# matchylabs/matchy

Hardware: AMD Instinct MI355X
Metric: log GB/s scanned (matchy match hot path, 100K IoCs) (higher is better)
Workload: dtype u8

## Files before the change

### matchy_amd/csrc/validate_kernels.hip

```cpp
#include <hip/hip_runtime.h>

#include <cstdlib>

#include "hashes.h"
#include "scan_types.h"

#include "device_shared.h"

namespace mxy {


struct BackReader {
    const uint8_t* p;
    uint32_t pos;
    uint32_t cb;
    uint32_t k;
    uint64_t cur, nxt;
    __device__ __forceinline__ static uint64_t load8(const uint8_t* a) { uint64_t v; __builtin_memcpy(&v, a, 8); return v; }
    __device__ __forceinline__ void init(const uint8_t* base, uint32_t q) {
        p = base; pos = q; cb = 0; k = 0; cur = 0; nxt = 0;
        if (q >= 16) { cb = q - 8; k = 8; cur = load8(p + cb); nxt = load8(p + cb - 8); }
    }
    __device__ __forceinline__ uint32_t next() {
        --pos;
        if (pos < 16) return p[pos];
        if (k == 0) { cur = nxt; cb -= 8; k = 8; nxt = cb >= 8 ? load8(p + cb - 8) : 0ull; }
        const uint32_t c = (uint32_t)(cur >> 56);
        cur <<= 8;
        --k;
        return c;
    }
};

struct WalkInit {
    uint64_t rh;
    uint32_t cur = 0, last_c = 0, labels = 1;
    bool high = false, bad = false, found = false;
};
struct WalkState { uint32_t pos, cur, last_c, labels; bool high, bad, found; };
constexpr int WALK_NO = 0, WALK_YES = 1, WALK_LONG = 2;
constexpr uint32_t WALK_BUDGET_WORDS = 128;
template <bool HASH>
__device__ __forceinline__ int domain_walk_back(const LogView& lg, const DevDb& db, uint32_t min_labels, uint32_t e, BackReader& br,
                                                 const WalkInit& wi, uint32_t& start, WalkState* long_out, bool* defer_utf8 = nullptr,
                                                 bool* hit_start = nullptr) {
    uint64_t rh = wi.rh;
    bool found = wi.found, bad = wi.bad, high = wi.high;
    uint32_t labels = wi.labels, cur = wi.cur, last_c = wi.last_c;
    uint32_t first_c = 0x100;
    uint32_t words = 0;
    while (br.pos > 0) {
        if ((!HASH || found) && br.pos >= 32 && (cur != 0 || last_c == '.')) {
            constexpr uint64_t H = 0x8080808080808080ull;
            uint32_t pos = br.pos;
            uint64_t w = BackReader::load8(lg.p + pos - 8);
            bool any = false;
            for (;;) {
                const uint64_t wn = pos >= 24 ? BackReader::load8(lg.p + pos - 16) : 0ull;
                const ByteMasks m = domain_masks(w);
                if ((~m.dc & H) != 0) break;
                const uint64_t dr = (m.dot >> 8) | (last_c == '.' ? (0x80ull << 56) : 0ull);
                const uint64_t sr = (m.dash >> 8) | (last_c == '-' ? (0x80ull << 56) : 0ull);
                if (((m.dot & (dr | sr)) | (m.dash & dr)) != 0) bad = true;
                if (m.dot != 0 && !bad) found = true;
                labels += (uint32_t)__popcll(m.dot);
                high |= m.high != 0;
                last_c = (uint32_t)w & 0xFF;
                cur = last_c == '.' ? 0u : 1u;
                pos -= 8;
                any = true;
                if (pos < 24) break;
                if (long_out && ++words >= WALK_BUDGET_WORDS) {
                    *long_out = WalkState{pos, cur, last_c, labels, high, bad, found};
                    return WALK_LONG;
                }
                w = wn;
            }
            if (any) { br.init(lg.p, pos); continue; }
        }
        uint32_t c = br.next();
        if (!d_is_domain_char_fast(c)) { first_c = c; ++br.pos; break; }
        if (HASH && !found && e - br.pos - 1 > db.max_suffix_len) return WALK_NO;
        if (c == '.') {
            if (cur == 0 || last_c == '-') bad = true;
            if (HASH) { if (!found && !bad) found = psl_contains(db, psl_hash_finish(rh), lg.p + br.pos + 1, e - br.pos - 1); }
            else if (!bad) found = true;
            ++labels;
            cur = 0;
        } else {
            if (cur == 0 && c == '-') bad = true;
            ++cur;
            high |= c >= 0x80;
        }
        if (HASH) rh = psl_hash_step(rh, (uint8_t)c);
        last_c = c;
    }
    const uint32_t s = br.pos;
    if (hit_start && first_c == 0x100) *hit_start = true;
    if (cur == 0 || last_c == '-') bad = true;
    if (bad || !found || labels < min_labels) return WALK_NO;
    if (first_c != 0x100 && !d_is_boundary(first_c)) return WALK_NO;
    if (high && defer_utf8) *defer_utf8 = true;
    else if (high && !d_valid_utf8(lg.p + s, e - s)) return WALK_NO;
    start = s;
    return WALK_YES;
}

__device__ __forceinline__ bool coop_valid_utf8(const uint8_t* p, uint32_t n) {
    const uint32_t lane = lane_id();
    uint64_t carry = 0;
    uint32_t c2 = 0;
    bool ok = true;
    for (uint32_t base = 0; base < n; base += 64) {
        const uint32_t b = base + lane < n ? p[base + lane] : 0u;
        const uint64_t cont = __ballot((b & 0xC0u) == 0x80u);
        const uint64_t l2 = __ballot(b >= 0xC2u && b <= 0xDFu), l3 = __ballot((b & 0xF0u) == 0xE0u), l4 = __ballot(b >= 0xF0u && b <= 0xF4u);
        const uint64_t badb = __ballot(b == 0xC0u || b == 0xC1u || b >= 0xF5u);
        const uint64_t e0 = __ballot(b == 0xE0u), ed = __ballot(b == 0xEDu), f0 = __ballot(b == 0xF0u), f4 = __ballot(b == 0xF4u);
        const uint64_t ltA0 = __ballot(b < 0xA0u), gt9F = __ballot(b > 0x9Fu), lt90 = __ballot(b < 0x90u), gt8F = __ballot(b > 0x8Fu);
        const uint64_t lead = l2 | l3 | l4, lead34 = l3 | l4;
        const uint64_t exp = (lead << 1) | (lead34 << 2) | (l4 << 3) | carry;
        carry = (lead >> 63) | (lead34 >> 62) | (l4 >> 61);
        uint64_t bad2 = ((e0 << 1) & ltA0) | ((ed << 1) & gt9F) | ((f0 << 1) & lt90) | ((f4 << 1) & gt8F);
        if (c2 & 1) bad2 |= ltA0 & 1; if (c2 & 2) bad2 |= gt9F & 1; if (c2 & 4) bad2 |= lt90 & 1; if (c2 & 8) bad2 |= gt8F & 1;
        c2 = (uint32_t)(e0 >> 63) | ((uint32_t)(ed >> 63) << 1) | ((uint32_t)(f0 >> 63) << 2) | ((uint32_t)(f4 >> 63) << 3);
        if ((exp ^ cont) | badb | bad2) { ok = false; break; }
    }
    return ok && carry == 0;
}

__device__ __forceinline__ void coop_domain_skip(const LogView& lg, WalkState& st) {
    constexpr uint64_t H = 0x8080808080808080ull;
    const uint32_t lane = lane_id();
    while (st.pos >= 512 + 32) {
        const uint32_t base = st.pos - 512;
        const uint64_t w = BackReader::load8(lg.p + base + 8 * lane);
        const ByteMasks m = domain_masks(w);
        const uint64_t stop = __ballot((~m.dc & H) != 0);
        const int hi = stop ? 63 - (int)__clzll((long long)stop) : -1;
        const bool valid = (int)lane > hi;
        uint32_t nb = (uint32_t)__shfl_down((int)((uint32_t)w & 0xFFu), 1);
        if (lane == 63) nb = st.last_c;
        const uint64_t dr = (m.dot >> 8) | (nb == '.' ? (0x80ull << 56) : 0ull);
        const uint64_t sr = (m.dash >> 8) | (nb == '-' ? (0x80ull << 56) : 0ull);
        const bool badl = ((m.dot & (dr | sr)) | (m.dash & dr)) != 0;
        if (__ballot(valid && badl)) st.bad = true;
        if (__ballot(valid && m.dot != 0) && !st.bad) st.found = true;
        if (__ballot(valid && m.high != 0)) st.high = true;
        uint32_t nd = valid ? (uint32_t)__popcll(m.dot) : 0u;
#pragma unroll
        for (int off = 32; off > 0; off >>= 1) nd += (uint32_t)__shfl_xor((int)nd, off);
        st.labels += nd;
        const uint32_t low = (uint32_t)w & 0xFFu;
        if (hi >= 0) {
            if (hi < 63) {
                st.pos = base + 8 * (uint32_t)(hi + 1);
                st.last_c = (uint32_t)__shfl((int)low, hi + 1);
                st.cur = st.last_c == '.' ? 0u : 1u;
            }
            return;
        }
        st.pos = base;
        st.last_c = (uint32_t)__shfl((int)low, 0);
        st.cur = st.last_c == '.' ? 0u : 1u;
    }
}

struct DomLong { WalkState st; uint32_t e; bool alone; };
__device__ int val_domain(const LogView& lg, const DevDb& db, const uint32_t* bloom, const uint2* tldtab, uint32_t min_labels,
                          uint32_t j, uint32_t& start, uint32_t& end, DomLong* long_out, bool* edge = nullptr) {
    uint32_t p = j, th = 2166136261u;
    bool open = true;
    uint32_t stop_c = 0x100;
    uint2 w = make_uint2(0u, 0u);
    const bool wide = j + 8 <= lg.len;
    if (wide) {
        __builtin_memcpy(&w, lg.p + j, 8);
#pragma unroll
        for (int k = 0; k < 8; ++k) {
            if (open) {
                const uint32_t c = ((k < 4 ? w.x : w.y) >> (8 * (k & 3))) & 0xFF;
                if (!d_is_domain_char_fast(c)) { open = false; stop_c = c; }
                else {
                    if (c == '.') return false;
                    th = tld_hash_step(th, c);
                    ++p;
                }
            }
        }
    }
    while (open && p < lg.len) {
        uint32_t c = lg.at(p);
        if (!d_is_domain_char_fast(c)) { stop_c = c; break; }
        if (c == '.') return false;
        if (p - j >= db.max_tld_len) return false;
        th = tld_hash_step(th, c);
        ++p;
    }
    const uint32_t e = p, ll = e - j;
    if (edge && stop_c == 0x100) *edge = true;
    if (ll > db.max_tld_len) return false;
    if (stop_c != 0x100 && !d_is_boundary(stop_c)) return false;
    bool alone = false;
    if (wide && ll <= 7) {
        const uint32_t lo = ll >= 4 ? w.x : (w.x & ((1u << (8 * ll)) - 1u));
        const uint32_t hi = ll > 4 ? (w.y & ((1u << (8 * (ll - 4))) - 1u)) : 0u;
        uint32_t slot = tld_tab_slot(lo, hi);
        for (;;) {
            const uint2 t = tldtab[slot];
            if ((t.y >> 24) == 0) return false;
            if (t.x == lo && (t.y & 0xFFFFFFu) == hi) { alone = (t.y >> 24) & 1; break; }
            slot = (slot + 1) & ((1u << TLD_TAB_BITS) - 1);
        }
    } else {
        const uint32_t bit = tld_hash_bit(th);
        if (!((bloom[bit >> 5] >> (bit & 31)) & 1)) return false;
    }
    uint32_t s;
    BackReader br;
    br.init(lg.p, e);
    WalkInit wi;
    wi.rh = psl_hash_init();
    WalkState ws{};
    const int r = alone ? domain_walk_back<false>(lg, db, min_labels, e, br, wi, s, long_out ? &ws : nullptr, nullptr, edge)
                        : domain_walk_back<true>(lg, db, min_labels, e, br, wi, s, long_out ? &ws : nullptr, nullptr, edge);
    if (r == WALK_LONG) { long_out->st = ws; long_out->e = e; long_out->alone = alone; return WALK_LONG; }
    if (r != WALK_YES) return WALK_NO;
    start = s; end = e;
    return WALK_YES;
}
__device__ bool val_domain_resume(const LogView& lg, const DevDb& db, uint32_t min_labels, const DomLong& dl, uint32_t& start, uint32_t& end, bool& need_utf8) {
    BackReader br;
    br.init(lg.p, dl.st.pos);
    WalkInit wi;
    wi.rh = psl_hash_init();
    wi.cur = dl.st.cur; wi.last_c = dl.st.last_c; wi.labels = dl.st.labels; wi.high = dl.st.high; wi.bad = dl.st.bad; wi.found = dl.st.found;
    uint32_t s;
    if (domain_walk_back<false>(lg, db, min_labels, dl.e, br, wi, s, nullptr, &need_utf8) != WALK_YES) return false;
    start = s; end = dl.e;
    return true;
}

__device__ __forceinline__ int val_domain_pre(const uint2* tldtab, uint32_t min_labels, uint32_t j, uint2 w, uint64_t b0, uint64_t b1,
                                              uint64_t b2, uint32_t& start, uint32_t& end) {
    constexpr uint64_t H = 0x8080808080808080ull;
    const uint64_t w64 = (uint64_t)w.x | ((uint64_t)w.y << 32);
    const ByteMasks mw = domain_masks(w64);
    const uint64_t ndc = ~mw.dc & H;
    const uint32_t ll = ndc ? (uint32_t)(__ffsll((long long)ndc) - 1) >> 3 : 8u;
    if (ll <= 7 && ll >= 1) {
        const uint64_t below = (1ull << (8 * ll)) - 1ull;
        if (mw.dot & below) return 0;
        const uint32_t stop_c = (uint32_t)(w64 >> (8 * ll)) & 0xFF;
        if (!d_is_boundary(stop_c)) return 0;
        const uint32_t lo = (uint32_t)(w64 & below), hi = (uint32_t)((w64 & below) >> 32);
        uint32_t slot = tld_tab_slot(lo, hi);
        bool alone = false;
        for (;;) {
            const uint2 t = tldtab[slot];
            if ((t.y >> 24) == 0) return 0;
            if (t.x == lo && (t.y & 0xFFFFFFu) == hi) { alone = (t.y >> 24) & 1; break; }
            slot = (slot + 1) & ((1u << TLD_TAB_BITS) - 1);
        }
        if (alone) {
            const ByteMasks m0 = domain_masks(b0), m1 = domain_masks(b1), m2 = domain_masks(b2);
            const uint64_t n0m = ~m0.dc & H, n1m = ~m1.dc & H, n2m = ~m2.dc & H;
            const uint32_t c0 = n0m ? (uint32_t)__clzll((long long)n0m) >> 3 : 8u;
            const uint32_t c1 = n1m ? (uint32_t)__clzll((long long)n1m) >> 3 : 8u, c2 = n2m ? (uint32_t)__clzll((long long)n2m) >> 3 : 8u;
            const uint32_t consumed = c0 < 8 ? c0 : (c1 < 8 ? 8 + c1 : 16 + c2);
            if (consumed < 24 || j == 24) {
                auto top = [](uint32_t k) -> uint64_t { return k == 0 ? 0ull : (~0ull << (64 - 8 * k)); };
                const uint64_t r0 = top(min(consumed, 8u)), r1 = top(consumed > 8 ? min(consumed - 8, 8u) : 0u),
                               r2 = top(consumed > 16 ? consumed - 16 : 0u);
                const uint64_t d0 = m0.dot >> 8, d1 = (m1.dot >> 8) | (m0.dot << 56), d2 = (m2.dot >> 8) | (m1.dot << 56);
                const uint64_t s0 = m0.dash >> 8, s1 = (m1.dash >> 8) | (m0.dash << 56), s2 = (m2.dash >> 8) | (m1.dash << 56);
                const uint64_t bad = ((m0.dot & (d0 | s0)) | (m0.dash & d0)) & r0;
                const uint64_t bad1 = ((m1.dot & (d1 | s1)) | (m1.dash & d1)) & r1, bad2 = ((m2.dot & (d2 | s2)) | (m2.dash & d2)) & r2;
                const uint32_t ndots = (uint32_t)(__popcll(m0.dot & r0) + __popcll(m1.dot & r1) + __popcll(m2.dot & r2));
                const uint32_t li = 24 - consumed;
                const uint64_t lw = li < 8 ? b2 : li < 16 ? b1 : b0;
                const uint32_t left_c = (uint32_t)(lw >> (8 * (li & 7))) & 0xFF;
                const uint32_t fi = 23 - consumed;
                const uint64_t fw = fi < 8 ? b2 : fi < 16 ? b1 : b0;
                const uint32_t first_c = consumed < 24 ? (uint32_t)(fw >> (8 * (fi & 7))) & 0xFF : 0x100u;
                const uint32_t lastc = (uint32_t)(w64 >> (8 * (ll - 1))) & 0xFF;
                const bool any_bad = (bad | bad1 | bad2) != 0 || lastc == '-' || consumed == 0 || left_c == '.' || left_c == '-';
                if (any_bad || ndots == 0 || 1 + ndots < min_labels) return 0;
                if (first_c != 0x100 && !d_is_boundary(first_c)) return 0;
                const uint32_t s_pos = j - consumed;
                const bool high = ((m0.high & r0) | (m1.high & r1) | (m2.high & r2) | (mw.high & below)) != 0;
                if (high) return 2;
                start = s_pos; end = j + ll;
                return 1;
            }
        }
    }
    return 2;
}

template <int NB>
__device__ __forceinline__ int val_domain_ctx(const uint2* tldtab, uint32_t min_labels, uint32_t j, uint2 w, const uint64_t (&b)[NB],
                                              uint32_t& start, uint32_t& end) {
    static_assert(NB >= 1 && NB <= 7, "a label must not reach 64 bytes inside the context");
    constexpr uint64_t H = 0x8080808080808080ull;
    const uint64_t w64 = (uint64_t)w.x | ((uint64_t)w.y << 32);
    const ByteMasks mw = domain_masks(w64);
    const uint64_t ndc = ~mw.dc & H;
    const uint32_t ll = ndc ? (uint32_t)(__ffsll((long long)ndc) - 1) >> 3 : 8u;
    if (ll > 7 || ll < 1) return 2;
    const uint64_t below = (1ull << (8 * ll)) - 1ull;
    if (mw.dot & below) return 0;
    const uint32_t stop_c = (uint32_t)(w64 >> (8 * ll)) & 0xFF;
    if (!d_is_boundary(stop_c)) return 0;
    const uint32_t lo = (uint32_t)(w64 & below), hi = (uint32_t)((w64 & below) >> 32);
    uint32_t slot = tld_tab_slot(lo, hi);
    bool alone = false;
    for (;;) {
        const uint2 t = tldtab[slot];
        if ((t.y >> 24) == 0) return 0;
        if (t.x == lo && (t.y & 0xFFFFFFu) == hi) { alone = (t.y >> 24) & 1; break; }
        slot = (slot + 1) & ((1u << TLD_TAB_BITS) - 1);
    }
    if (!alone) return 2;
    ByteMasks m[NB];
    uint32_t consumed = 0;
    bool open = true;
#pragma unroll
    for (int k = 0; k < NB; ++k) {
        m[k] = domain_masks(b[k]);
        const uint64_t nm = ~m[k].dc & H;
        const uint32_t ck = nm ? (uint32_t)__clzll((long long)nm) >> 3 : 8u;
        if (open) { consumed += ck; open = ck == 8; }
    }
    if (consumed == 8 * NB && j != 8 * NB) return 2;
    uint64_t bad = 0, high = mw.high & below;
    uint32_t ndots = 0;
#pragma unroll
    for (int k = 0; k < NB; ++k) {
        const uint32_t in_k = consumed > 8u * k ? min(consumed - 8u * k, 8u) : 0u;
        const uint64_t r = in_k == 0 ? 0ull : (~0ull << (64 - 8 * in_k));
        const uint64_t d = (m[k].dot >> 8) | (k ? (m[k ? k - 1 : 0].dot << 56) : 0ull);
        const uint64_t sd = (m[k].dash >> 8) | (k ? (m[k ? k - 1 : 0].dash << 56) : 0ull);
        bad |= ((m[k].dot & (d | sd)) | (m[k].dash & d)) & r;
        ndots += (uint32_t)__popcll(m[k].dot & r);
        high |= m[k].high & r;
    }
    const uint32_t li = 8 * NB - consumed, fi = li - 1;
    uint32_t left_c = 0, first_c = 0x100u;
#pragma unroll
    for (int k = 0; k < NB; ++k) {
        const uint32_t wi = (uint32_t)(NB - 1 - k);
        if ((li >> 3) == wi) left_c = (uint32_t)(b[k] >> (8 * (li & 7))) & 0xFF;
        if (consumed < 8 * NB && (fi >> 3) == wi) first_c = (uint32_t)(b[k] >> (8 * (fi & 7))) & 0xFF;
    }
    const uint32_t lastc = (uint32_t)(w64 >> (8 * (ll - 1))) & 0xFF;
    const bool any_bad = bad != 0 || lastc == '-' || consumed == 0 || left_c == '.' || left_c == '-';
    if (any_bad || ndots == 0 || 1 + ndots < min_labels) return 0;
    if (first_c != 0x100u && !d_is_boundary(first_c)) return 0;
    if (high) return 2;
    start = j - consumed; end = j + ll;
    return 1;
}

__device__ bool all_hex(const LogView& lg, uint32_t s, uint32_t n) {
    for (uint32_t k = 0; k < n; ++k) if (!d_is_hex(lg.at(s + k))) return false;
    return true;
}
__device__ __forceinline__ bool hex4(uint32_t x) {
    const uint32_t t = x & 0x7F7F7F7Fu, l = t | 0x20202020u;
    const uint32_t dig = (t + 0x50505050u) & ~(t + 0x46464646u);
    const uint32_t alp = (l + 0x1F1F1F1Fu) & ~(l + 0x19191919u);
    return (((dig | alp) & ~x) & 0x80808080u) == 0x80808080u;
}
__device__ __forceinline__ bool all_hex_wide(const uint8_t* p, uint32_t n) {
    bool ok = true;
#pragma unroll 4
    for (uint32_t k = 0; k < n; k += 8) {
        uint2 v;
        __builtin_memcpy(&v, p + k, 8);
        ok = ok && hex4(v.x) && hex4(v.y);
    }
    return ok;
}


__device__ __forceinline__ uint32_t d_lower(uint32_t c) { return (c - 'A' < 26u) ? c + 32 : c; }

__device__ bool val_ipv6(const LogView& lg, uint32_t p2, uint32_t& start, uint32_t& end) {
    uint32_t s = p2 - 1;
    while (s > 0) { uint32_t c = lg.at(s - 1); if (!d_is_hex(c) && c != ':') break; --s; }
    uint32_t e = p2 + 1;
    while (e < lg.len) { uint32_t c = lg.at(e); if (!d_is_hex(c) && c != ':') break; ++e; }
    uint32_t n = e - s;
    if (n < 8 || n > 64) return false;
    const uint8_t* c = lg.p + s;
    if ((c[0] == ':' && c[1] == ':') || (c[n - 2] == ':' && c[n - 1] == ':')) return false;
    if (d_lower(c[0]) == 'f' && d_lower(c[1]) == 'e') { uint32_t x = d_lower(c[2]); if (x == '8' || x == '9' || x == 'a' || x == 'b') return false; }
    uint16_t seg[8];
    if (!d_parse_ipv6(c, n, seg)) return false;
    start = s; end = e;
    return true;
}

__device__ bool val_ipv6_win(const uint8_t* win, uint32_t p2, uint32_t& start, uint32_t& end) {
    uint32_t s = 39;
    while (s > 0) { uint32_t c = win[s - 1]; if (!d_is_hex(c) && c != ':') break; --s; }
    if (s == 0) return false;
    uint32_t e = 41;
    while (e < 80) { uint32_t c = win[e]; if (!d_is_hex(c) && c != ':') break; ++e; }
    if (e == 80) return false;
    const uint32_t n = e - s;
    if (n < 8 || n > 64) return false;
    const uint8_t* c = win + s;
    if ((c[0] == ':' && c[1] == ':') || (c[n - 2] == ':' && c[n - 1] == ':')) return false;
    if (d_lower(c[0]) == 'f' && d_lower(c[1]) == 'e') { uint32_t x = d_lower(c[2]); if (x == '8' || x == '9' || x == 'a' || x == 'b') return false; }
    uint16_t seg[8];
    if (!d_parse_ipv6(c, n, seg)) return false;
    start = p2 - 40 + s; end = p2 - 40 + e;
    return true;
}

struct LocalMasks { uint64_t loc, dot, alp; };
struct LocalMasks32 { uint32_t loc, dot, alp; };
__device__ __forceinline__ LocalMasks32 email_local_masks32(uint32_t x) {
    constexpr uint32_t H = 0x80808080u, L7 = 0x7F7F7F7Fu;
    const uint32_t t = x & L7, l = t | 0x20202020u;
    const uint32_t dig = (t + 0x50505050u) & ~(t + 0x46464646u);
    const uint32_t alp = (l + 0x1F1F1F1Fu) & ~(l + 0x05050505u);
    const uint32_t ndot = (t ^ 0x2E2E2E2Eu) + L7, ndash = (t ^ 0x2D2D2D2Du) + L7;
    const uint32_t nus = (t ^ 0x5F5F5F5Fu) + L7, npl = (t ^ 0x2B2B2B2Bu) + L7;
    LocalMasks32 m;
    m.dot = ~ndot & ~x & H;
    m.alp = alp & ~x & H;
    m.loc = (dig | alp | ~ndot | ~ndash | ~nus | ~npl) & ~x & H;
    return m;
}
__device__ __forceinline__ LocalMasks email_local_masks(uint64_t x) {
    const LocalMasks32 lo = email_local_masks32((uint32_t)x), hi = email_local_masks32((uint32_t)(x >> 32));
    LocalMasks m;
    m.loc = (uint64_t)lo.loc | ((uint64_t)hi.loc << 32);
    m.dot = (uint64_t)lo.dot | ((uint64_t)hi.dot << 32);
    m.alp = (uint64_t)lo.alp | ((uint64_t)hi.alp << 32);
    return m;
}
struct EmailState { uint32_t s, prev; bool has_letter, dotdot; };
__device__ __forceinline__ bool email_local_scan(const LogView& lg, EmailState& es, bool budget) {
    constexpr uint64_t H = 0x8080808080808080ull;
    uint32_t s = es.s, prev = es.prev, words = 0;
    bool has_letter = es.has_letter, dotdot = es.dotdot, is_long = false;
    if (s >= 32) {
        uint64_t w = BackReader::load8(lg.p + s - 8);
        for (;;) {
// ... 237 lines not shown
            const uint64_t t = bc[(i + 4) % 5] ^ rotl64(bc[(i + 1) % 5], 1);
#pragma unroll
            for (int j = 0; j < 25; j += 5) st[j + i] ^= t;
        }
        uint64_t t = st[1];
#pragma unroll
        for (int i = 0; i < 24; ++i) { const int j = PILN[i]; const uint64_t b = st[j]; st[j] = rotl64(t, ROTC[i]); t = b; }
#pragma unroll
        for (int j = 0; j < 25; j += 5) {
#pragma unroll
            for (int i = 0; i < 5; ++i) bc[i] = st[j + i];
#pragma unroll
            for (int i = 0; i < 5; ++i) st[j + i] ^= (~bc[(i + 1) % 5]) & bc[(i + 2) % 5];
        }
        st[0] ^= RC[round];
    }
    out[0] = st[0]; out[1] = st[1]; out[2] = st[2]; out[3] = st[3];
}

__device__ __forceinline__ int d_b58_val(uint32_t c) {
    if (c >= '1' && c <= '9') return (int)c - '1';
    if (c >= 'A' && c <= 'H') return (int)c - 'A' + 9;
    if (c >= 'J' && c <= 'N') return (int)c - 'J' + 17;
    if (c >= 'P' && c <= 'Z') return (int)c - 'P' + 22;
    if (c >= 'a' && c <= 'k') return (int)c - 'a' + 33;
    if (c >= 'm' && c <= 'z') return (int)c - 'm' + 44;
    return -1;
}
template <int NL>
__device__ uint32_t d_base58_decode(const uint8_t* s, uint32_t n, uint8_t* dec) {
    uint32_t L[NL];
#pragma unroll
    for (int i = 0; i < NL; ++i) L[i] = 0;
    uint32_t zeros = 0;
    bool leading = true;
    for (uint32_t k = 0; k < n; ++k) {
        const int v = d_b58_val(s[k]);
        if (v < 0) return 0;
        if (leading && v == 0) { ++zeros; continue; }
        leading = false;
        uint32_t carry = (uint32_t)v;
#pragma unroll
        for (int i = 0; i < NL; ++i) {
            const uint64_t t = (uint64_t)L[i] * 58u + carry;
            L[i] = (uint32_t)t;
            carry = (uint32_t)(t >> 32);
        }
    }
    uint32_t nbytes = 0;
#pragma unroll
    for (int i = 0; i < NL; ++i) if (L[i]) nbytes = 4 * i + 1 + ((31u - (uint32_t)__clz((int)L[i])) >> 3);
    for (uint32_t k = 0; k < zeros; ++k) dec[k] = 0;
#pragma unroll
    for (int i = 0; i < NL; ++i) {
#pragma unroll
        for (int bb = 0; bb < 4; ++bb) {
            const uint32_t j = 4 * i + bb;
            if (j < nbytes) dec[zeros + nbytes - 1 - j] = (uint8_t)(L[i] >> (8 * bb));
        }
    }
    return zeros + nbytes;
}
__device__ bool val_btc_base58(const uint8_t* s, uint32_t n, uint8_t* dec) {
    const uint32_t dl = d_base58_decode<12>(s, n, dec);
    if (dl < 5) return false;
    Sha256 h1, h2;
    h1.hash(dec, dl - 4);
    uint32_t w[16];
#pragma unroll
    for (int i = 0; i < 8; ++i) w[i] = h1.h[i];
    w[8] = 0x80000000u;
#pragma unroll
    for (int i = 9; i < 15; ++i) w[i] = 0;
    w[15] = 256;
    h2.init();
    h2.block(w);
    const uint32_t chk = ((uint32_t)dec[dl - 4] << 24) | ((uint32_t)dec[dl - 3] << 16) | ((uint32_t)dec[dl - 2] << 8) | dec[dl - 1];
    return h2.h[0] == chk;
}
__device__ bool val_monero(const uint8_t* s, uint32_t n, uint8_t* dec) {
    const uint32_t dl = d_base58_decode<21>(s, n, dec);
    if (dl < 5) return false;
    uint64_t h[4];
    d_keccak256_1blk(dec, dl - 4, h);
    const uint32_t chk = (uint32_t)dec[dl - 4] | ((uint32_t)dec[dl - 3] << 8) | ((uint32_t)dec[dl - 2] << 16) | ((uint32_t)dec[dl - 1] << 24);
    return (uint32_t)h[0] == chk;
}
__device__ int d_bech32_val(uint32_t c) {
    const char* CS = "qpzry9x8gf2tvdw0s3jn54khce6mua7l";
    for (int i = 0; i < 32; ++i) if ((uint32_t)CS[i] == c) return i;
    return -1;
}
__device__ bool val_btc_bech32(const uint8_t* s, uint32_t n) {
    if (n < 3 + 6) return false;
    auto step = [](uint32_t chk, uint32_t v) {
        const uint32_t GEN[5] = {0x3b6a57b2, 0x26508e6d, 0x1ea119fa, 0x3d4233dd, 0x2a1462b3};
        uint32_t top = chk >> 25;
        chk = ((chk & 0x1ffffff) << 5) ^ v;
        for (int i = 0; i < 5; ++i) if ((top >> i) & 1) chk ^= GEN[i];
        return chk;
    };
    uint32_t chk = 1;
    chk = step(chk, 'b' >> 5); chk = step(chk, 'c' >> 5); chk = step(chk, 0); chk = step(chk, 'b' & 31); chk = step(chk, 'c' & 31);
    for (uint32_t k = 3; k < n; ++k) {
        int v = d_bech32_val(s[k]);
        if (v < 0) return false;
        chk = step(chk, (uint32_t)v);
    }
    return chk == 1 || chk == 0x2bc830a3u;
}
__device__ bool val_eth(const uint8_t* a, uint8_t* lower) {
    bool all_lower = true, all_upper = true;
    for (int i = 0; i < 40; ++i) {
        uint32_t c = a[2 + i];
        if (!d_is_hex(c)) return false;
        if (d_is_alpha(c)) { if (c >= 'a') all_upper = false; else all_lower = false; }
        lower[i] = (uint8_t)d_lower(c);
    }
    if (all_lower || all_upper) return true;
    uint64_t h[4];
    d_keccak256_1blk(lower, 40, h);
    for (int i = 0; i < 40; ++i) {
        uint32_t c = a[2 + i];
        if (d_is_alpha(c)) {
            const uint32_t byte = (uint32_t)(h[i >> 4] >> (8 * ((i >> 1) & 7))) & 0xFF;
            const uint32_t nib = (i & 1) ? (byte & 0x0f) : (byte >> 4);
            if ((c < 'a') != (nib >= 8)) return false;
        }
    }
    return true;
}

template <int MODE>
__global__ __launch_bounds__(256) void k_validate_dom(TokParams p, DevDb db) {
    constexpr bool AC = MODE == 1, SFX = MODE == 2;
    __shared__ uint2 tldtab[1u << TLD_TAB_BITS];
    __shared__ __attribute__((aligned(16))) uint32_t strbuf[256][8];
    __shared__ uint8_t dcls[AC ? 256 : 4];
    __shared__ uint32_t drows[AC ? DFA_LDS_ENTRIES_VAL : 1];
    for (uint32_t i = threadIdx.x; i < (1u << TLD_TAB_BITS); i += blockDim.x) tldtab[i] = db.tld_tab[i];
    DfaView dv{dcls, drows, 0};
    if constexpr (AC) dv = dfa_stage<DFA_LDS_ENTRIES_VAL>(db, dcls, drows);
    __syncthreads();
    ChunkWriter<Candidate, CAND_CHUNK> cw_dense;
    __shared__ Candidate wb_cand[4][64];
    BufferedWriter<Candidate> cw(wb_cand[threadIdx.x >> 6]);
    __shared__ RareAnchor wb_slow[4][64];
    BufferedWriter<RareAnchor> sw(wb_slow[threadIdx.x >> 6]);
    const Candidate SC{0, 0xFFFFFFFFu, 0, 0};
    const uint32_t stride = gridDim.x * blockDim.x;
    const uint32_t nd = min(p.counters->n_dom, p.dom_cap);
    struct Rec { uint32_t j; uint32_t c[8]; };
    auto load_rec = [&](uint32_t i, Rec& r) {
        r.j = 0xFFFFFFFFu;
#pragma unroll
        for (int k = 0; k < 8; ++k) r.c[k] = 0;
        if (i < nd) {
            r.j = p.dom_list[dom_plane_index(i, 0)];
#pragma unroll
            for (int k = 0; k < 8; ++k) r.c[k] = p.dom_list[dom_plane_index(i, 1 + k)];
        }
    };
    Rec cur, nxt;
    load_rec(blockIdx.x * blockDim.x + threadIdx.x, cur);
    {
        uint32_t g = cur.j;
#pragma unroll
        for (int k = 0; k < 8; ++k) g ^= cur.c[k];
        asm volatile("" ::"v"(g));
    }
    uint32_t pend_start = 0, pend_lt = 0, pend_word = 0xFFFFFFFFu, pend_bit = 0, n_valid = 0;
    uint32_t pend_sw[SFX ? 4 : 1] = {0}, pend_sb[SFX ? 4 : 1] = {0};
    bool pend = false, pend_over = false;
    uint32_t* sb = strbuf[threadIdx.x];
    auto queue_glob = [&](uint32_t b, uint32_t n) {
        if (!p.glob_work_d) return;
        const uint32_t lane = lane_id();
        const bool g = lane < n && b + lane < p.cand_cap && cw.buf[lane].pad == CAND_GLOB;
        const uint64_t m = __ballot(g);
        if (!m) return;
        uint32_t wb = 0;
        if (lane == 0) wb = atomicAdd(&p.counters->n_glob_work_d, (uint32_t)__popcll(m));
        wb = __builtin_amdgcn_readfirstlane(wb);
        const uint32_t slot = wb + mbcnt64(m);
        if (g && slot < p.glob_work_d_cap) p.glob_work_d[slot] = b + lane;
    };
    auto emit_pending = [&]() {
        if (!p.filter_lit) { cw_dense.append(pend, Candidate{pend_start, pend_lt, 0u, 0u}, p.cands, p.cand_cap, p.n_cand, SC); return; }
        bool lit = (pend_word >> pend_bit) & 1;
        uint32_t flag = 0;
        if constexpr (SFX) {
            bool g = pend_over;
#pragma unroll
            for (int q = 0; q < 4; ++q) g = g || ((pend_sw[q] >> pend_sb[q]) & 1);
            flag = g ? CAND_GLOB : CAND_NO_GLOB;
            lit = lit || g;
        }
        if constexpr (AC) flag = pend_over ? CAND_GLOB : CAND_NO_GLOB;
        if constexpr (AC || SFX) cw.append_then(pend && lit, Candidate{pend_start, pend_lt, 0u, flag}, p.cands, p.cand_cap, p.n_cand, queue_glob);
        else cw.append(pend && lit, Candidate{pend_start, pend_lt, 0u, flag}, p.cands, p.cand_cap, p.n_cand);
    };
    for (uint32_t base = blockIdx.x * blockDim.x; base < nd; base += stride) {
        const uint32_t i = base + threadIdx.x;
        emit_pending();
        pend = false;
        load_rec(i + stride, nxt);
        bool slow = false;
        if (cur.j != 0xFFFFFFFFu) {
            uint32_t s = 0, e = 0;
            int r = 2;
            if (!(cur.j & 0x80000000u)) {
                const uint64_t b2 = (uint64_t)cur.c[0] | ((uint64_t)cur.c[1] << 32), b1 = (uint64_t)cur.c[2] | ((uint64_t)cur.c[3] << 32),
                               b0 = (uint64_t)cur.c[4] | ((uint64_t)cur.c[5] << 32);
                r = val_domain_pre(tldtab, p.min_labels, cur.j, make_uint2(cur.c[6], cur.c[7]), b0, b1, b2, s, e);
            }
            slow = r == 2;
            if (r == 1) {
                pend_start = s; pend_lt = (e - s) | ((uint32_t)IT_DOMAIN << 24); pend = true;
                pend_word = 0xFFFFFFFFu; pend_bit = 0;
                n_valid += 1;
                if (p.filter_lit) {
                    *reinterpret_cast<uint4*>(sb) = make_uint4(cur.c[0], cur.c[1], cur.c[2], cur.c[3]);
                    *reinterpret_cast<uint4*>(sb + 4) = make_uint4(cur.c[4], cur.c[5], cur.c[6], cur.c[7]);
                    const uint32_t o = 24 - (cur.j - s), n = e - s;
                    const uint32_t i0 = o >> 2, sh = o & 3;
                    uint32_t wd[9];
#pragma unroll
                    for (int k = 0; k < 9; ++k) wd[k] = (i0 + k) < 8 ? sb[(i0 + k) & 7] : 0u;
                    uint64_t ln[4];
#pragma unroll
                    for (int k = 0; k < 4; ++k)
                        ln[k] = (uint64_t)__builtin_amdgcn_alignbyte(wd[2 * k + 1], wd[2 * k], sh) |
                                ((uint64_t)__builtin_amdgcn_alignbyte(wd[2 * k + 2], wd[2 * k + 1], sh) << 32);
                    if (db.ci) {
#pragma unroll
                        for (int k = 0; k < 4; ++k) ln[k] = ascii_lower8(ln[k]);
                    }
                    const uint32_t b = name_hash31(ln[0], ln[1], ln[2], ln[3], n) & db.lit_bm_mask;
                    pend_word = db.lit_bm ? db.lit_bm[b >> 5] : 0u;
                    pend_bit = b & 31;
                    if constexpr (SFX) {
                        const uint64_t fb = 0x0101010101010101ull * db.sfx_first;
                        uint32_t M = 0;
#pragma unroll
                        for (int k = 0; k < 4; ++k) {
                            const uint64_t x = ln[k] ^ fb;
                            const uint64_t z = ~(((x & 0x7F7F7F7F7F7F7F7Full) + 0x7F7F7F7F7F7F7F7Full) | x) & 0x8080808080808080ull;
                            const uint32_t lo = (uint32_t)z >> 7, hi = (uint32_t)(z >> 32) >> 7;
                            M |= ((((lo * 0x01020408u) >> 24) & 0xFu) | ((((hi * 0x01020408u) >> 24) & 0xFu) << 4)) << (8 * k);
                        }
                        M &= n >= 32 ? 0xFFFFFFFFu : ((1u << n) - 1u);
                        pend_over = false;
                        uint32_t dm = db.sfx_dots;
#pragma unroll
                        for (int q = 0; q < 4; ++q) {
                            pend_sw[q] = 0; pend_sb[q] = 0;
                            if (dm) {
                                const uint32_t d = (uint32_t)__builtin_ctz(dm) + 1;
                                dm &= dm - 1;
                                uint32_t m = M;
                                for (uint32_t j = 1; j < d; ++j) m &= ~(m ? (0x80000000u >> __builtin_clz(m)) : 0u);
                                if (m) {
                                    const uint32_t kk = 31u - (uint32_t)__builtin_clz(m), sl = n - kk;
                                    if (sl >= 3) {
                                        const uint32_t o2 = o + kk, j0 = o2 >> 2, s2 = o2 & 3;
                                        uint32_t w2[9];
#pragma unroll
                                        for (int k = 0; k < 9; ++k) w2[k] = (j0 + k) < 8 ? sb[(j0 + k) & 7] : 0u;
                                        uint64_t l2[4];
#pragma unroll
                                        for (int k = 0; k < 4; ++k)
                                            l2[k] = (uint64_t)__builtin_amdgcn_alignbyte(w2[2 * k + 1], w2[2 * k], s2) |
                                                    ((uint64_t)__builtin_amdgcn_alignbyte(w2[2 * k + 2], w2[2 * k + 1], s2) << 32);
                                        if (db.ci) {
#pragma unroll
                                            for (int k = 0; k < 4; ++k) l2[k] = ascii_lower8(l2[k]);
                                        }
                                        const uint32_t b2 = name_hash31(l2[0], l2[1], l2[2], l2[3], sl) & db.sfx_mask;
                                        pend_sw[q] = db.sfx_bm[b2 >> 5];
                                        pend_sb[q] = b2 & 31;
                                    }
                                }
                            }
                        }
                    }
                    if constexpr (AC) {
                        uint32_t st = 0, any = 0;
#pragma unroll
                        for (int k = 0; k < 31; ++k) {
                            const uint32_t c = dcls[(uint32_t)(ln[k >> 3] >> (8 * (k & 7))) & 0xFF];
                            if ((uint32_t)k < n) {
                                const uint32_t t = st < dv.lds_states ? drows[st * db.dfa_k + c] : db.dfa[(size_t)st * db.dfa_k + c];
                                st = t & 0x7FFFFFFFu;
                                any |= t;
                            }
                        }
                        pend_over = (any >> 31) != 0;
                        if (pend_over) { pend_word = 0xFFFFFFFFu; pend_bit = 0; }
                    }
                }
            }
        }
        sw.append(slow, RareAnchor{cur.j & 0x7FFFFFFFu, (uint32_t)RARE_DOM}, p.rare_dom, p.rare_dom_cap, &p.counters->n_rare_dom);
        cur = nxt;
    }
    emit_pending();
    if constexpr (AC || SFX) cw.flush_then(p.cands, p.cand_cap, p.n_cand, queue_glob);
    else cw.flush(p.cands, p.cand_cap, p.n_cand);
    cw_dense.pad_rest(p.cands, p.cand_cap, SC);
    sw.flush(p.rare_dom, p.rare_dom_cap, &p.counters->n_rare_dom);
#pragma unroll
    for (int off = 32; off > 0; off >>= 1) n_valid += __shfl_down(n_valid, off);
    if (lane_id() == 0 && n_valid) atomicAdd(&p.counters->cand_true, n_valid);
}

__device__ __forceinline__ bool lit_bm_may_hit(const DevDb& db, const LogView& lg, uint32_t s, uint32_t n, bool ascii) {
    uint64_t l[4] = {0, 0, 0, 0};
    if (s + 32 <= lg.len) {
#pragma unroll
        for (int k = 0; k < 4; ++k) __builtin_memcpy(&l[k], lg.p + s + 8 * k, 8);
    } else {
        for (uint32_t k = 0; k < 32 && s + k < lg.len; ++k) l[k >> 3] |= (uint64_t)lg.p[s + k] << (8 * (k & 7));
    }
    if (db.ci) {
        if (!ascii) {
            if (n > 32) return true;
            uint64_t high = 0;
#pragma unroll
            for (int k = 0; k < 4; ++k) {
                const int rem = (int)n - 8 * k;
                const uint64_t m = rem >= 8 ? ~0ull : (rem <= 0 ? 0ull : ((1ull << (8 * rem)) - 1ull));
                high |= l[k] & m & 0x8080808080808080ull;
            }
            if (high) return true;
        }
#pragma unroll
        for (int k = 0; k < 4; ++k) l[k] = ascii_lower8(l[k]);
    }
    const uint32_t b = name_hash31(l[0], l[1], l[2], l[3], n) & db.lit_bm_mask;
    return ((db.lit_bm[b >> 5] >> (b & 31)) & 1u) != 0;
}

template <uint32_t VM>
__global__ __launch_bounds__(256) void k_validate(TokParams p, DevDb db) {
    constexpr bool MISC = (VM & 1u) != 0, DOM = (VM & 2u) != 0, TOK = (VM & 4u) != 0;
    __shared__ uint32_t bloom[DOM ? TLD_BLOOM_WORDS : 1];
    constexpr bool TLD_LDS = DOM && (MISC || TOK);
    __shared__ uint2 tldtab[TLD_LDS ? (1u << TLD_TAB_BITS) : 1];
    const uint2* const tldtab_p = TLD_LDS ? tldtab : db.tld_tab;
    constexpr uint32_t WIN = MISC ? 80 : 64;
    constexpr uint32_t WIN_BACK = WIN - (MISC ? 32 : 16);
    __shared__ __attribute__((aligned(16))) uint8_t winbuf[(MISC || DOM) ? 256 * WIN : 16];
    if constexpr (DOM && !MISC && !TOK) {
        if (blockIdx.x * blockDim.x >= min(p.counters->n_rare_dom, p.rare_dom_cap)) return;
    }
    if constexpr (TOK && !MISC && !DOM) {
        if (blockIdx.x * blockDim.x >= min(p.counters->n_tok, p.tok_cap)) return;
    }
    if constexpr (DOM) {
        for (uint32_t i = threadIdx.x; i < TLD_BLOOM_WORDS; i += blockDim.x) bloom[i] = db.tld_bloom[i];
        if constexpr (TLD_LDS) for (uint32_t i = threadIdx.x; i < (1u << TLD_TAB_BITS); i += blockDim.x) tldtab[i] = db.tld_tab[i];
        __syncthreads();
    }
    LogView lg{p.log, p.len};
    __shared__ Candidate wb_cand[4][64];
    BufferedWriter<Candidate> cw(wb_cand[threadIdx.x >> 6]);
    const uint32_t stride = gridDim.x * blockDim.x;
    __shared__ RareAnchor wb_heavy[4][64];
// ... 336 lines not shown
```

Measured before the change: 2301.

## Validate domain candidates with bit-transposed context planes instead of per-word byte masks

Replaces the per-64-bit-word byte-mask domain validation with a bit-plane version: the 32-byte context is permuted and bit-transposed so each character class becomes a 32-bit mask, and label, run and boundary checks become single-word bit operations. The TLD hash probe now happens after the branch-free run checks instead of gating them. Record loading is also made unconditional by clamping the index, which removes divergent branches around the global loads. The transpose adds fixed ALU work per candidate and may compute more than the old early-exit path did for rejected candidates.

```diff
diff --git a/matchy_amd/csrc/domain_planes.h b/matchy_amd/csrc/domain_planes.h
--- /dev/null
+++ b/matchy_amd/csrc/domain_planes.h
@@ -0,0 +1,89 @@
+#pragma once
+#include <cstdint>
+
+#include "anchor_planes.h"
+
+namespace mxy {
+
+MXY_HD uint32_t byte_perm(uint32_t hi, uint32_t lo, uint32_t sel) {
+#if defined(__HIP_DEVICE_COMPILE__)
+    return __builtin_amdgcn_perm(hi, lo, sel);
+#else
+    const uint64_t v = ((uint64_t)hi << 32) | lo;
+    uint32_t r = 0;
+    for (int k = 0; k < 4; ++k) r |= (uint32_t)((v >> (8 * ((sel >> (8 * k)) & 7u))) & 0xFFu) << (8 * k);
+    return r;
+#endif
+}
+
+struct ContextMasks {
+    uint32_t DC;
+    uint32_t DOT;
+    uint32_t DASH;
+    uint32_t HIGH;
+    uint32_t B;
+};
+
+MXY_HD ContextMasks context_planes(const uint32_t (&c)[8]) {
+    uint32_t w[8];
+#pragma unroll
+    for (int h = 0; h < 2; ++h) {
+        const uint32_t alo = byte_perm(c[h + 2], c[h], 0x05010400u), ahi = byte_perm(c[h + 2], c[h], 0x07030602u);
+        const uint32_t blo = byte_perm(c[h + 6], c[h + 4], 0x05010400u), bhi = byte_perm(c[h + 6], c[h + 4], 0x07030602u);
+        w[4 * h + 0] = byte_perm(blo, alo, 0x05040100u);
+        w[4 * h + 1] = byte_perm(blo, alo, 0x07060302u);
+        w[4 * h + 2] = byte_perm(bhi, ahi, 0x05040100u);
+        w[4 * h + 3] = byte_perm(bhi, ahi, 0x07060302u);
+    }
+    bit_transpose8(w);
+    const ClassPlanes k = classify_planes(w, true);
+    ContextMasks m;
+    m.DC = k.TL | k.T;
+    m.DOT = k.T;
+    m.DASH = andn(k.LD, k.TL);
+    m.HIGH = w[7];
+    m.B = k.B;
+    return m;
+}
+
+MXY_HD uint32_t dp_ctz(uint32_t x) { return (uint32_t)__builtin_ctz(x); }
+MXY_HD uint32_t dp_clz(uint32_t x) { return (uint32_t)__builtin_clz(x); }
+MXY_HD uint32_t dp_popc(uint32_t x) { return (uint32_t)__builtin_popcount(x); }
+
+template <class Slot>
+MXY_HD int domain_rules(const Slot* tldtab, uint32_t min_labels, uint32_t j, const uint32_t (&c)[8], uint32_t& start, uint32_t& end) {
+    const ContextMasks m = context_planes(c);
+    const uint32_t ndc = ~m.DC >> 24;
+    const uint32_t ll = ndc ? dp_ctz(ndc) : 8u;
+    const uint32_t label = ((1u << ll) - 1u) << 24;
+    const uint32_t consumed = dp_clz(~(m.DC << 8));
+    const uint32_t li = 24 - consumed;
+    const uint32_t r = (0xFFFFFFFFu << li) & 0x00FFFFFFu;
+    const uint32_t D = m.DOT & 0x00FFFFFFu, S = m.DASH & 0x00FFFFFFu;
+    const uint32_t bad = ((D & ((D | S) >> 1)) | (S & (D >> 1))) & r;
+    const uint32_t ndots = dp_popc(D & r);
+    const uint32_t edge = (((D | S) >> li) | (m.DASH >> (23 + ll))) & 1u;
+    const uint32_t front = ((m.B << 1) >> li) & 1u;
+    const bool whole = consumed == 24;
+    const bool no_name = ((bad | edge) != 0) | (consumed == 0) | (ndots == 0) | (1 + ndots < min_labels) | (!whole & (front == 0));
+    const bool high = (m.HIGH & (r | label)) != 0;
+    const int by_run = (whole & (j != 24)) ? 2 : no_name ? 0 : high ? 2 : 1;
+    const bool no_label = ((m.DOT & label) != 0) | ((((m.B >> 24) >> ll) & 1u) == 0);
+    if (ll > 7 || ll < 1) return 2;
+    if (no_label) return 0;
+    const uint32_t lo = ll >= 4 ? c[6] : c[6] & ((1u << (8 * ll)) - 1u);
+    const uint32_t hi = ll > 4 ? c[7] & ((1u << (8 * ll - 32)) - 1u) : 0u;
+    uint32_t slot = tld_tab_slot(lo, hi);
+    bool alone = false;
+    for (;;) {
+        const Slot t = tldtab[slot];
+        if ((t.y >> 24) == 0) return 0;
+        if (t.x == lo && (t.y & 0xFFFFFFu) == hi) { alone = (t.y >> 24) & 1; break; }
+        slot = (slot + 1) & ((1u << TLD_TAB_BITS) - 1);
+    }
+    if (!alone) return 2;
+    start = j - consumed; end = j + ll;
+    return by_run;
+}
+
+}
diff --git a/matchy_amd/csrc/validate_kernels.hip b/matchy_amd/csrc/validate_kernels.hip
--- a/matchy_amd/csrc/validate_kernels.hip
+++ b/matchy_amd/csrc/validate_kernels.hip
@@ -6,6 +6,7 @@
 #include "scan_types.h"
 
 #include "device_shared.h"
+#include "domain_planes.h"
 
 namespace mxy {
 
@@ -241,63 +242,6 @@
     return true;
 }
 
-__device__ __forceinline__ int val_domain_pre(const uint2* tldtab, uint32_t min_labels, uint32_t j, uint2 w, uint64_t b0, uint64_t b1,
-                                              uint64_t b2, uint32_t& start, uint32_t& end) {
-    constexpr uint64_t H = 0x8080808080808080ull;
-    const uint64_t w64 = (uint64_t)w.x | ((uint64_t)w.y << 32);
-    const ByteMasks mw = domain_masks(w64);
-    const uint64_t ndc = ~mw.dc & H;
-    const uint32_t ll = ndc ? (uint32_t)(__ffsll((long long)ndc) - 1) >> 3 : 8u;
-    if (ll <= 7 && ll >= 1) {
-        const uint64_t below = (1ull << (8 * ll)) - 1ull;
-        if (mw.dot & below) return 0;
-        const uint32_t stop_c = (uint32_t)(w64 >> (8 * ll)) & 0xFF;
-        if (!d_is_boundary(stop_c)) return 0;
-        const uint32_t lo = (uint32_t)(w64 & below), hi = (uint32_t)((w64 & below) >> 32);
-        uint32_t slot = tld_tab_slot(lo, hi);
-        bool alone = false;
-        for (;;) {
-            const uint2 t = tldtab[slot];
-            if ((t.y >> 24) == 0) return 0;
-            if (t.x == lo && (t.y & 0xFFFFFFu) == hi) { alone = (t.y >> 24) & 1; break; }
-            slot = (slot + 1) & ((1u << TLD_TAB_BITS) - 1);
-        }
-        if (alone) {
-            const ByteMasks m0 = domain_masks(b0), m1 = domain_masks(b1), m2 = domain_masks(b2);
-            const uint64_t n0m = ~m0.dc & H, n1m = ~m1.dc & H, n2m = ~m2.dc & H;
-            const uint32_t c0 = n0m ? (uint32_t)__clzll((long long)n0m) >> 3 : 8u;
-            const uint32_t c1 = n1m ? (uint32_t)__clzll((long long)n1m) >> 3 : 8u, c2 = n2m ? (uint32_t)__clzll((long long)n2m) >> 3 : 8u;
-            const uint32_t consumed = c0 < 8 ? c0 : (c1 < 8 ? 8 + c1 : 16 + c2);
-            if (consumed < 24 || j == 24) {
-                auto top = [](uint32_t k) -> uint64_t { return k == 0 ? 0ull : (~0ull << (64 - 8 * k)); };
-                const uint64_t r0 = top(min(consumed, 8u)), r1 = top(consumed > 8 ? min(consumed - 8, 8u) : 0u),
-                               r2 = top(consumed > 16 ? consumed - 16 : 0u);
-                const uint64_t d0 = m0.dot >> 8, d1 = (m1.dot >> 8) | (m0.dot << 56), d2 = (m2.dot >> 8) | (m1.dot << 56);
-                const uint64_t s0 = m0.dash >> 8, s1 = (m1.dash >> 8) | (m0.dash << 56), s2 = (m2.dash >> 8) | (m1.dash << 56);
-                const uint64_t bad = ((m0.dot & (d0 | s0)) | (m0.dash & d0)) & r0;
-                const uint64_t bad1 = ((m1.dot & (d1 | s1)) | (m1.dash & d1)) & r1, bad2 = ((m2.dot & (d2 | s2)) | (m2.dash & d2)) & r2;
-                const uint32_t ndots = (uint32_t)(__popcll(m0.dot & r0) + __popcll(m1.dot & r1) + __popcll(m2.dot & r2));
-                const uint32_t li = 24 - consumed;
-                const uint64_t lw = li < 8 ? b2 : li < 16 ? b1 : b0;
-                const uint32_t left_c = (uint32_t)(lw >> (8 * (li & 7))) & 0xFF;
-                const uint32_t fi = 23 - consumed;
-                const uint64_t fw = fi < 8 ? b2 : fi < 16 ? b1 : b0;
-                const uint32_t first_c = consumed < 24 ? (uint32_t)(fw >> (8 * (fi & 7))) & 0xFF : 0x100u;
-                const uint32_t lastc = (uint32_t)(w64 >> (8 * (ll - 1))) & 0xFF;
-                const bool any_bad = (bad | bad1 | bad2) != 0 || lastc == '-' || consumed == 0 || left_c == '.' || left_c == '-';
-                if (any_bad || ndots == 0 || 1 + ndots < min_labels) return 0;
-                if (first_c != 0x100 && !d_is_boundary(first_c)) return 0;
-                const uint32_t s_pos = j - consumed;
-                const bool high = ((m0.high & r0) | (m1.high & r1) | (m2.high & r2) | (mw.high & below)) != 0;
-                if (high) return 2;
-                start = s_pos; end = j + ll;
-                return 1;
-            }
-        }
-    }
-    return 2;
-}
-
 template <int NB>
 __device__ __forceinline__ int val_domain_ctx(const uint2* tldtab, uint32_t min_labels, uint32_t j, uint2 w, const uint64_t (&b)[NB],
                                               uint32_t& start, uint32_t& end) {
@@ -841,14 +785,11 @@
     const uint32_t nd = min(p.counters->n_dom, p.dom_cap);
     struct Rec { uint32_t j; uint32_t c[8]; };
     auto load_rec = [&](uint32_t i, Rec& r) {
-        r.j = 0xFFFFFFFFu;
-#pragma unroll
-        for (int k = 0; k < 8; ++k) r.c[k] = 0;
-        if (i < nd) {
-            r.j = p.dom_list[dom_plane_index(i, 0)];
-#pragma unroll
-            for (int k = 0; k < 8; ++k) r.c[k] = p.dom_list[dom_plane_index(i, 1 + k)];
-        }
+        const uint32_t ic = i < nd ? i : 0u;
+        const uint32_t j = p.dom_list[dom_plane_index(ic, 0)];
+#pragma unroll
+        for (int k = 0; k < 8; ++k) r.c[k] = p.dom_list[dom_plane_index(ic, 1 + k)];
+        r.j = i < nd ? j : 0xFFFFFFFFu;
     };
     Rec cur, nxt;
     load_rec(blockIdx.x * blockDim.x + threadIdx.x, cur);
@@ -898,11 +839,7 @@
         if (cur.j != 0xFFFFFFFFu) {
             uint32_t s = 0, e = 0;
             int r = 2;
-            if (!(cur.j & 0x80000000u)) {
-                const uint64_t b2 = (uint64_t)cur.c[0] | ((uint64_t)cur.c[1] << 32), b1 = (uint64_t)cur.c[2] | ((uint64_t)cur.c[3] << 32),
-                               b0 = (uint64_t)cur.c[4] | ((uint64_t)cur.c[5] << 32);
-                r = val_domain_pre(tldtab, p.min_labels, cur.j, make_uint2(cur.c[6], cur.c[7]), b0, b1, b2, s, e);
-            }
+            if (!(cur.j & 0x80000000u)) r = domain_rules(tldtab, p.min_labels, cur.j, cur.c, s, e);
             slow = r == 2;
             if (r == 1) {
                 pend_start = s; pend_lt = (e - s) | ((uint32_t)IT_DOMAIN << 24); pend = true;
```

New measurement: 2334 (median of 6 runs). 1.01x the previous value.
